# ribal-aladeeb/reinforcement-learning-2048

Measured on AMD Instinct MI355X. Metric: 2048 env steps/sec + DQN updates/sec at 64k parallel boards, 1→8 MI355X, higher is better.
Workload: dtype u8

## Files before the change

reinforcement-learning-2048_amd/csrc/g2048_learn64.hip:

```cpp
#include <hip/hip_runtime.h>
#include <math.h>
#include <stdint.h>
#include <stdlib.h>

#include "../../include/g2048.h"
#include "g2048_board.hpp"
#include "g2048_common.hpp"

namespace {

constexpr int NT = 256;
constexpr int S = 64;
constexpr int XS = 17;
constexpr int HS = 65;
constexpr int P_W1 = 0, P_B1 = 1024, P_W2 = 1088, P_B2 = 1344, P_N = 1348;
constexpr int SLAB = P_N + 4;
constexpr int MAX_SLABS = 256;

struct Net64 {
    double *w1, *b1, *w2, *b2;
};

struct alignas(16) Smem {
    double x[S * XS];
    double h[S * HS];
    double w2[2][4 * 64];
    double b1[2][64];
    double b2[2][4];
    double qa[S * 4];
    double qb[S * 4];
    double y[S];
    double dq[S];
    double loss[S];
    int act[S];
};

__device__ __forceinline__ int64_t sample_row(int64_t b, unsigned long long ep,
                                              unsigned long long count, uint32_t lo, uint32_t hi) {
    const uint4 u = g2048::philox10(
        make_uint4((uint32_t)b, (uint32_t)((uint64_t)b >> 32), (uint32_t)ep,
                   (uint32_t)(ep >> 32) | (g2048::DOMAIN_SAMPLE << 30)),
        lo, hi);
    return (int64_t)__umul64hi(((unsigned long long)u.y << 32) | u.x, count);
}

__device__ __forceinline__ void put_row(double* xr, uint4 v) {
    const uint32_t w[4] = {v.x, v.y, v.z, v.w};
#pragma unroll
    for (int k = 0; k < 4; ++k) {
        xr[4 * k + 0] = (double)(w[k] & 0xFFu);
        xr[4 * k + 1] = (double)((w[k] >> 8) & 0xFFu);
        xr[4 * k + 2] = (double)((w[k] >> 16) & 0xFFu);
        xr[4 * k + 3] = (double)(w[k] >> 24);
    }
}

__device__ __forceinline__ void forward(Smem& M, const double (&w1r)[16], int net, double* q) {
    const int t = threadIdx.x, j = t & 63, rq = t >> 6;
    const double bj = M.b1[net][j];
#pragma unroll 4
    for (int rr = 0; rr < 16; ++rr) {
        const int s = rq * 16 + rr;
        const double* xr = M.x + s * XS;
        double acc = 0.0;
#pragma unroll
        for (int k = 0; k < 16; ++k) acc = fma(w1r[k], xr[k], acc);
        const double pre = acc + bj;
        M.h[s * HS + j] = pre > 0.0 ? pre : 0.0;
    }
    __syncthreads();
    const int s = t >> 2, a = t & 3;
    const double* hr = M.h + s * HS;
    const double* w2 = M.w2[net] + a * 64;
    double acc = 0.0;
#pragma unroll 8
    for (int jj = 0; jj < 64; ++jj) acc = fma(w2[jj], hr[jj], acc);
    q[s * 4 + a] = acc + M.b2[net][a];
    __syncthreads();
}

struct UpdArgs64 {
    Net64 on, tg;
    const uint4 *s, *s2;
    const uint8_t *a, *d;
    const int32_t* r;
    const unsigned long long* count;
    const unsigned long long* step;
    const int64_t* idx_in;
    int64_t batch;
    uint32_t seed_lo, seed_hi;
    float gamma;
    int double_dqn;
    int64_t* idx_out;
    double* y_out;
    double* slab;
    unsigned long long* step_next;
};

typedef uint32_t u32x2 __attribute__((ext_vector_type(2)));
constexpr int AUX_SC1 = 16;
__device__ __forceinline__ __amdgpu_buffer_rsrc_t slab_rsrc(const double* base) {
    return __builtin_amdgcn_make_buffer_rsrc(const_cast<double*>(base), 0, 0x7FFFFFFF, 0x00020000);
}
template <bool COH>
__device__ __forceinline__ void slab_put(double* sl, int e, double v) {
    if constexpr (COH)
        __builtin_amdgcn_raw_buffer_store_b64(__builtin_bit_cast(u32x2, v), slab_rsrc(sl),
                                              (uint32_t)e * 8u, 0u, AUX_SC1);
    else
        sl[e] = v;
}

template <bool COH>
__device__ __forceinline__ void update_tiles64(const UpdArgs64& A) {
    __shared__ Smem M;
    const int t = threadIdx.x, j = t & 63, qd = t >> 6;
    const unsigned long long ep = A.idx_in ? 0ull : *A.step;
    const unsigned long long count = A.idx_in ? 0ull : *A.count;
    if (blockIdx.x == 0 && t == 0) *A.step_next = *A.step + 1ull;
    const Net64 nets[2] = {A.tg, A.on};
    double w1t[16], w1o[16];
#pragma unroll
    for (int k = 0; k < 16; ++k) {
        w1t[k] = A.tg.w1[j * 16 + k];
        w1o[k] = A.on.w1[j * 16 + k];
    }
    for (int i = t; i < 2 * 256; i += NT) M.w2[i >> 8][i & 255] = nets[i >> 8].w2[i & 255];
    if (t < 128) M.b1[t >> 6][t & 63] = nets[t >> 6].b1[t & 63];
    if (t < 8) M.b2[t >> 2][t & 3] = nets[t >> 2].b2[t & 3];
    double w2o[4];
#pragma unroll
    for (int a = 0; a < 4; ++a) w2o[a] = A.on.w2[a * 64 + j];
    double g_w1[4] = {0.0, 0.0, 0.0, 0.0}, g_b1 = 0.0, g_w2 = 0.0, g_b2 = 0.0, g_loss = 0.0;
    const int64_t ntiles = (A.batch + S - 1) / S;
    for (int64_t tile = blockIdx.x; tile < ntiles; tile += gridDim.x) {
        const int64_t b = tile * S + t;
        uint4 sv = make_uint4(0u, 0u, 0u, 0u);
        double rj = 0.0;
        float disc = 0.f;
        bool ok = false;
        __syncthreads();
        if (t < S) {
            uint4 s2v = make_uint4(0u, 0u, 0u, 0u);
            int aj = 0;
            ok = b < A.batch;
            if (ok) {
                const int64_t row =
                    A.idx_in ? A.idx_in[b] : sample_row(b, ep, count, A.seed_lo, A.seed_hi);
                A.idx_out[b] = row;
                s2v = A.s2[row];
                sv = A.s[row];
                aj = A.a[row];
                rj = (double)A.r[row];
                disc = (float)(1 - (int)A.d[row]) * A.gamma;
            }
            put_row(M.x + t * XS, s2v);
            M.act[t] = aj;
        }
        __syncthreads();
        forward(M, w1t, 0, M.qa);
        forward(M, w1o, 1, M.qb);
        if (t < S) {
            const double* qo = M.qb + t * 4;
            const double* qt = M.qa + t * 4;
            double next;
            if (A.double_dqn) {
                const uint32_t as = g2048::argmax4_torch(qo[0], qo[1], qo[2], qo[3]);
                next = qt[as];
            } else {
                next = g2048::qmax4_torch(qt[0], qt[1], qt[2], qt[3]);
            }
            double y;
            {
#pragma clang fp contract(off)
                y = rj + (double)disc * next;
            }
            M.y[t] = y;
            if (ok) A.y_out[b] = y;
            put_row(M.x + t * XS, sv);
        }
        __syncthreads();
        forward(M, w1o, 1, M.qb);
        if (t < S) {
            double dq = 0.0, l = 0.0;
            if (ok) {
#pragma clang fp contract(off)
                const double e = M.qb[t * 4 + M.act[t]] - M.y[t];
                dq = 2.0 * e;
                l = e * e;
            }
            M.dq[t] = dq;
            M.loss[t] = l;
        }
        __syncthreads();
        {
            double acc = 0.0, accb = 0.0;
            for (int s = 0; s < S; ++s) {
                if (M.act[s] == qd) {
                    acc = fma(M.dq[s], M.h[s * HS + j], acc);
                    accb += M.dq[s];
                }
            }
            g_w2 += acc;
            if (j == 0) g_b2 += accb;
        }
        if (t == 0) {
            double l = 0.0;
            for (int s = 0; s < S; ++s) l += M.loss[s];
            g_loss += l;
        }
        __syncthreads();
#pragma unroll 4
        for (int rr = 0; rr < 16; ++rr) {
            const int s = qd * 16 + rr;
            double& hv = M.h[s * HS + j];
            const double w = M.act[s] == 0 ? w2o[0] : M.act[s] == 1 ? w2o[1]
                           : M.act[s] == 2 ? w2o[2] : w2o[3];
            hv = hv > 0.0 ? M.dq[s] * w : 0.0;
        }
        __syncthreads();
        {
            double acc[4] = {0.0, 0.0, 0.0, 0.0}, accb = 0.0;
            for (int s = 0; s < S; ++s) {
                const double dh = M.h[s * HS + j];
                const double* xr = M.x + s * XS + 4 * qd;
#pragma unroll
                for (int i = 0; i < 4; ++i) acc[i] = fma(dh, xr[i], acc[i]);
                accb += dh;
            }
#pragma unroll
            for (int i = 0; i < 4; ++i) g_w1[i] += acc[i];
            if (qd == 0) g_b1 += accb;
        }
    }
    double* sl = A.slab + (int64_t)blockIdx.x * SLAB;
#pragma unroll
    for (int i = 0; i < 4; ++i) slab_put<COH>(sl, P_W1 + j * 16 + 4 * qd + i, g_w1[i]);
    if (qd == 0) slab_put<COH>(sl, P_B1 + j, g_b1);
    slab_put<COH>(sl, P_W2 + qd * 64 + j, g_w2);
    if (j == 0) slab_put<COH>(sl, P_B2 + qd, g_b2);
    if (t == 0) slab_put<COH>(sl, P_N, g_loss);
}

__global__ __launch_bounds__(NT) void k_dense64_update_f64(UpdArgs64 A) { update_tiles64<false>(A); }

constexpr int RW = 16;
static_assert(MAX_SLABS <= RW * 16, "reduction covers at most RW*16 slabs");

struct RedArgs64 {
    const double* slab;
    int nslab;
    double* grad;
    double* loss;
    const unsigned long long* step_next;
    unsigned long long* step;
    double* p[4];
    double* tp[4];
    unsigned long long sync_every;
    double* m;
    double* v;
    double lr, b1, b2, eps;
    int adam;
};

template <int NW, bool COH>
__device__ __forceinline__ void reduce_positions64(const RedArgs64& A, int chunk,
                                                   unsigned long long t, double (*part)[64]) {
    const int lane = threadIdx.x & 63, wave = threadIdx.x >> 6;
    const int pos = chunk * 64 + lane;
    const int k = pos < P_B1 ? 0 : pos < P_W2 ? 1 : pos < P_B2 ? 2 : 3;
    const int base[4] = {P_W1, P_B1, P_W2, P_B2};
    const bool adam = A.adam && wave == 0 && pos < P_N;
    double am = 0.0, av = 0.0, ap = 0.0;
    if (adam) {
        am = A.m[pos];
        av = A.v[pos];
        ap = A.p[k][pos - base[k]];
    }
    constexpr int PW = RW / NW;
    const bool okp = pos <= P_N;
    const int pc = okp ? pos : P_N;
    double v[PW][16];
#pragma unroll
    for (int i = 0; i < PW; ++i)
#pragma unroll
        for (int u = 0; u < 16; ++u) {
            const int g = wave + NW * i + RW * u;
            const bool ok = okp && g < A.nslab;
            const int64_t e = (int64_t)(g < A.nslab ? g : 0) * SLAB + pc;
            double x;
            if constexpr (COH)
                x = __builtin_bit_cast(double, __builtin_amdgcn_raw_buffer_load_b64(
                                                   slab_rsrc(A.slab), (uint32_t)(e * 8), 0u, AUX_SC1));
            else
                x = A.slab[e];
            v[i][u] = ok ? x : 0.0;
        }
#pragma unroll
    for (int i = 0; i < PW; ++i) {
        double r = 0.0;
#pragma unroll
        for (int u = 0; u < 16; ++u) r += v[i][u];
        part[wave + NW * i][lane] = r;
    }
    __syncthreads();
    if (wave == 0 && pos <= P_N) {
        double sum = part[0][lane];
        for (int j = 1; j < RW; ++j) sum += part[j][lane];
        if (pos == P_N) {
            if (A.loss) *A.loss = sum;
        } else {
            if (A.grad) A.grad[pos] = sum;
            if (adam) {
                const double np = g2048::adam64((double)t, A.lr, A.b1, A.b2, A.eps, sum, am, av, ap);
                A.m[pos] = am;
                A.v[pos] = av;
                A.p[k][pos - base[k]] = np;
                if (A.sync_every && t % A.sync_every == 0ull) A.tp[k][pos - base[k]] = np;
            }
        }
    }
}

constexpr int RCHUNKS = (P_N + 1 + 63) / 64;

__global__ __launch_bounds__(64 * RW) void k_dense64_reduce_f64(RedArgs64 A) {
    __shared__ double part[RW][64];
    reduce_positions64<RW, false>(A, blockIdx.x, A.adam ? *A.step_next : 0ull, part);
    if (A.step && blockIdx.x == 0 && threadIdx.x == 0) *A.step = *A.step_next;
}

struct Upd1Args64 {
    UpdArgs64 U;
    RedArgs64 R;
    unsigned int* arrive;
};

__global__ __launch_bounds__(NT) void k_dense64_update1_f64(Upd1Args64 A) {
    const unsigned long long t_next = *A.U.step + 1ull;
    update_tiles64<true>(A.U);
    __shared__ unsigned int s_arrival;
    __shared__ double part[RW][64];
    const unsigned grid = gridDim.x;
    __builtin_amdgcn_s_waitcnt(0);
    __syncthreads();
    if (threadIdx.x == 0)
        s_arrival = __hip_atomic_fetch_add(&A.arrive[0], 1u, __ATOMIC_RELAXED,
                                           __HIP_MEMORY_SCOPE_AGENT);
    __syncthreads();
    const unsigned a = s_arrival;
    const unsigned nred = grid < (unsigned)RCHUNKS ? grid : (unsigned)RCHUNKS;
    if (a >= grid) {
        if (threadIdx.x == 0) atomicAdd(&A.arrive[2], 1u);
        return;
    }
    if (a < grid - nred) return;
    const unsigned me = a - (grid - nred);
    if (threadIdx.x == 0) {
        unsigned it = 0;
        while (__hip_atomic_load(&A.arrive[0], __ATOMIC_RELAXED, __HIP_MEMORY_SCOPE_AGENT) < grid) {
            __builtin_amdgcn_s_sleep(1);
            if (++it == (1u << 24)) {
                atomicAdd(&A.arrive[2], 1u);
                break;
            }
        }
    }
    __syncthreads();
    for (unsigned c = me; c < (unsigned)RCHUNKS; c += nred) {
        reduce_positions64<NT / 64, true>(A.R, (int)c, t_next, part);
        __syncthreads();
    }
    if (threadIdx.x == 0) {
        if (me == 0 && A.R.step) *A.R.step = t_next;
        if (__hip_atomic_fetch_add(&A.arrive[1], 1u, __ATOMIC_RELAXED, __HIP_MEMORY_SCOPE_AGENT) ==
            nred - 1) {
            __hip_atomic_store(&A.arrive[0], 0u, __ATOMIC_RELAXED, __HIP_MEMORY_SCOPE_AGENT);
            __hip_atomic_store(&A.arrive[1], 0u, __ATOMIC_RELAXED, __HIP_MEMORY_SCOPE_AGENT);
        }
    }
}

}

extern "C" G2048_API int64_t g2048_dense64_update_f64_workspace(int64_t batch) {
    const int64_t tiles = (batch + S - 1) / S;
    const int64_t grid = tiles < MAX_SLABS ? tiles : MAX_SLABS;
    return grid * SLAB + 1 + 2;
}

extern "C" G2048_API int g2048_dense64_update_f64(
    const g2048_dense64_params_f64* online, const g2048_dense64_params_f64* target,
    g2048_replay* rb, const int64_t* idx_in, int64_t batch, uint64_t seed, uint64_t* step_dev,
    float gamma, int double_dqn, int64_t* idx_out, double* y_out, double* workspace,
    double* grad_out, double* loss_out, double* exp_avg, double* exp_avg_sq, double lr,
    double beta1, double beta2, double eps, uint64_t sync_every, void* stream) {
    if (!online || !target || !rb || batch <= 0 || !step_dev || !idx_out || !y_out || !workspace)
        return g2048_fail(G2048_EINVAL, "dense64_update_f64: NULL argument or batch <= 0");
    if (!online->w1 || !online->b1 || !online->w2 || !online->b2 || !target->w1 || !target->b1 ||
        !target->w2 || !target->b2)
        return g2048_fail(G2048_EINVAL, "dense64_update_f64: NULL parameter pointer");
    const bool adam = exp_avg && exp_avg_sq;
    if (!adam && !grad_out)
        return g2048_fail(G2048_EINVAL,
                          "dense64_update_f64: need exp_avg and exp_avg_sq (Adam) or grad_out");
    uint8_t *s = nullptr, *s2 = nullptr, *a = nullptr, *d = nullptr;
    int32_t* r = nullptr;
    uint64_t* count = nullptr;
    if (g2048_replay_views(rb, &s, &s2, &a, &r, &d, &count) != G2048_OK) return G2048_EINVAL;
    const int64_t tiles = (batch + S - 1) / S;
    const int grid = (int)(tiles < MAX_SLABS ? tiles : MAX_SLABS);
    UpdArgs64 U;
    U.on = Net64{online->w1, online->b1, online->w2, online->b2};
    U.tg = Net64{target->w1, target->b1, target->w2, target->b2};
    U.s = reinterpret_cast<const uint4*>(s);
    U.s2 = reinterpret_cast<const uint4*>(s2);
    U.a = a;
    U.d = d;
    U.r = r;
    U.count = reinterpret_cast<const unsigned long long*>(count);
    U.step = reinterpret_cast<const unsigned long long*>(step_dev);
    U.idx_in = idx_in;
    U.batch = batch;
    U.seed_lo = (uint32_t)seed;
    U.seed_hi = (uint32_t)(seed >> 32);
    U.gamma = gamma;
    U.double_dqn = double_dqn;
    U.idx_out = idx_out;
    U.y_out = y_out;
    U.slab = workspace;
    U.step_next = reinterpret_cast<unsigned long long*>(workspace + (int64_t)grid * SLAB);
    hipStream_t st = reinterpret_cast<hipStream_t>(stream);
    RedArgs64 R;
    R.slab = workspace;
    R.nslab = grid;
    R.grad = grad_out;
    R.loss = loss_out;
    R.step_next = U.step_next;
    R.step = reinterpret_cast<unsigned long long*>(step_dev);
    double* ps[4] = {online->w1, online->b1, online->w2, online->b2};
    double* ts[4] = {target->w1, target->b1, target->w2, target->b2};
    for (int k = 0; k < 4; ++k) {
        R.p[k] = ps[k];
        R.tp[k] = ts[k];
    }
    R.sync_every = adam ? sync_every : 0ull;
    R.m = exp_avg;
    R.v = exp_avg_sq;
    R.lr = lr;
    R.b1 = beta1;
    R.b2 = beta2;
    R.eps = eps;
    R.adam = adam ? 1 : 0;
    const char* one = getenv("G2048_DENSE64_ONE_LAUNCH");
    if (one && one[0] == '1') {
        Upd1Args64 A1;
        A1.U = U;
        A1.R = R;
        A1.arrive = reinterpret_cast<unsigned int*>(U.step_next + 1);
        hipLaunchKernelGGL(k_dense64_update1_f64, dim3(grid), dim3(NT), 0, st, A1);
    } else {
        hipLaunchKernelGGL(k_dense64_update_f64, dim3(grid), dim3(NT), 0, st, U);
        hipLaunchKernelGGL(k_dense64_reduce_f64, dim3(RCHUNKS), dim3(64 * RW), 0, st, R);
    }
    const hipError_t e = hipGetLastError();
    return e == hipSuccess ? G2048_OK
                           : g2048_fail(G2048_EHIP, "dense64_update_f64: %s", hipGetErrorString(e));
// ... 2 lines not shown
```

reinforcement-learning-2048_amd/csrc/g2048_mlp.hip:

```cpp
#include <hip/hip_runtime.h>
#include <stdint.h>
#include <stdlib.h>

#include "../../include/g2048.h"
#include "g2048_board.hpp"
#include "g2048_common.hpp"

namespace {

constexpr int NT = 256, H = 64;
constexpr int XS = 20, W1S = 17, HS = 68, W2S = 68;
constexpr int S_FWD = 64;
constexpr int S_UPD = 32;
constexpr int P_W1 = 0, P_B1 = 1024, P_W2 = 1088, P_B2 = 1344, P_N = 1348;
constexpr int SLAB = 1352;
constexpr int MAX_SLABS = 256;

struct MlpW {
    const float *w1, *b1, *w2, *b2;
};

struct alignas(16) LW {
    float w1[H * W1S];
    float b1[H];
// ... 342 lines not shown
}

struct UpdateArgs {
    MlpW on, tg;
    const uint8_t *s, *a, *s2, *d;
    const int32_t* r;
    const unsigned long long* count;
    const unsigned long long* step;
    const int64_t* idx_in;
    int64_t batch;
    uint32_t seed_lo, seed_hi;
    float gamma;
    int double_dqn;
    int64_t* idx_out;
    float* y_out;
    float* slab;
    unsigned long long* step_next;
#ifdef G2048_MLP_PHASE
    long long* phase;
#endif
};

#ifdef G2048_MLP_PHASE
#define MPHASE(k) \
    if (threadIdx.x == 0) A.phase[blockIdx.x * 8 + (k)] = __builtin_amdgcn_s_memtime()
#else
#define MPHASE(k)
#endif

template <bool COH>
__device__ __forceinline__ void update_tiles(const UpdateArgs& A) {
    constexpr int S = S_UPD;
    MPHASE(0);
    __shared__ LW Won, Wtg;
    __shared__ Tile<S> T;
    __shared__ float qtg[S * 4];
    const int t = threadIdx.x;
    const unsigned long long ep = A.idx_in ? 0ull : *A.step;
    const unsigned long long count = A.idx_in ? 0ull : *A.count;
    if (blockIdx.x == 0 && t == 0) *A.step_next = *A.step + 1ull;
    stage_weights(A.on, Won);
    stage_weights(A.tg, Wtg);
    const float4 w1on = w1_lane(A.on), w1tg = w1_lane(A.tg);
    GradAcc G;
    const int64_t ntiles = (A.batch + S - 1) / S;
    const int sl = t >> 2, w = t & 3;
    for (int64_t tile = blockIdx.x; tile < ntiles; tile += gridDim.x) {
        const int64_t b0 = tile * S;
        const int64_t b = b0 + sl;
        const bool ok = t < 4 * S && b < A.batch;
        uint32_t s2w = 0, sw = 0;
        int32_t rj = 0;
        uint8_t dj = 0, aj = 0;
        if (ok) {
            const int64_t j =
                A.idx_in ? A.idx_in[b] : sample_row(b, ep, count, A.seed_lo, A.seed_hi);
            s2w = reinterpret_cast<const uint32_t*>(A.s2)[j * 4 + w];
            sw = reinterpret_cast<const uint32_t*>(A.s)[j * 4 + w];
            if (w == 0) {
                A.idx_out[b] = j;
                rj = A.r[j];
                dj = A.d[j];
                aj = A.a[j];
            }
        }
        __syncthreads();
        MPHASE(1);
        if (t < 4 * S) {
            put_word(T.x + sl * XS + w * 4, s2w);
            if (w == 0) {
                T.a[sl] = (float)aj;
                T.g[sl] = ok ? 1.f : 0.f;
            }
        }
        __syncthreads();
        MPHASE(2);
        forward_tile_mfma<S>(T, Wtg, w1tg);
        if (t < 4 * S) qtg[t] = T.q[t];
        forward_tile_mfma<S>(T, Won, w1on);
        if (t < 4 * S && w == 0) {
            const float y = bellman(T.q + sl * 4, qtg + sl * 4, rj, dj, A.gamma, A.double_dqn);
            T.y[sl] = y;
            if (ok) A.y_out[b] = y;
        }
        __syncthreads();
        MPHASE(3);
        if (t < 4 * S) put_word(T.x + sl * XS + w * 4, sw);
        __syncthreads();
        MPHASE(4);
        grad_tile<S>(T, Won, w1on, G);
#ifdef G2048_MLP_PHASE
        __syncthreads();
#endif
        MPHASE(5);
    }
    write_slab<S, COH>(G, T, A.slab + (int64_t)blockIdx.x * SLAB);
    MPHASE(6);
}

__global__ __launch_bounds__(NT) void k_mlp_update(UpdateArgs A) { update_tiles<false>(A); }

constexpr int RW = 16;
static_assert(MAX_SLABS <= RW * 16, "reduction covers at most RW*16 slabs");

struct ReduceArgs {
    const float* slab;
    int nslab;
    float* grad;
    float* loss;
    const unsigned long long* step_next;
    unsigned long long* step;
    float* p[4];
    float* tp[4];
    unsigned long long sync_every;
    float* m;
    float* v;
    double lr, b1, b2, eps;
    int adam;
};

template <int NW, bool COH>
__device__ __forceinline__ void reduce_positions(const ReduceArgs& A, int chunk,
                                                 unsigned long long t, float (*part)[64]) {
    const int lane = threadIdx.x & 63, wave = threadIdx.x >> 6;
    const int pos = chunk * 64 + lane;
    const bool adam = A.adam && wave == 0 && pos < P_N;
    const int k = pos < P_B1 ? 0 : pos < P_W2 ? 1 : pos < P_B2 ? 2 : 3;
    const int base[4] = {P_W1, P_B1, P_W2, P_B2};
    float am = 0.f, av = 0.f, ap = 0.f;
    if (adam) {
        am = A.m[pos];
        av = A.v[pos];
        ap = A.p[k][pos - base[k]];
    }
    constexpr int PW = RW / NW;
    const bool okp = pos <= P_N;
    const int pc = okp ? pos : P_N;
    float r[PW][16];
#pragma unroll
    for (int i = 0; i < PW; ++i)
#pragma unroll
        for (int u = 0; u < 16; ++u) {
            const int g = wave + NW * i + RW * u;
            const bool ok = okp && g < A.nslab;
            const int64_t e = (int64_t)(g < A.nslab ? g : 0) * SLAB + pc;
            float x;
            if constexpr (COH)
                x = __builtin_bit_cast(float, __builtin_amdgcn_raw_buffer_load_b32(
                                                  slab_rsrc(A.slab), (uint32_t)(e * 4), 0u, AUX_SC1));
            else
                x = A.slab[e];
            r[i][u] = ok ? x : 0.f;
        }
#pragma unroll
    for (int i = 0; i < PW; ++i) {
        float v = r[i][0];
#pragma unroll
        for (int u = 1; u < 16; ++u) v += r[i][u];
        part[wave + NW * i][lane] = v;
    }
    __syncthreads();
    if (wave == 0 && pos <= P_N) {
        float sum = part[0][lane];
#pragma unroll
        for (int k2 = 1; k2 < RW; ++k2) sum += part[k2][lane];
        if (pos == P_N) {
            if (A.loss) *A.loss = sum;
        } else {
            if (A.grad) A.grad[pos] = sum;
            if (adam) {
                const g2048::AdamCoef c = g2048::adam_coef((double)t, A.lr, A.b1, A.b2, A.eps);
                const float np = g2048::adam_update(c, sum, am, av, ap);
                A.m[pos] = am;
                A.v[pos] = av;
                A.p[k][pos - base[k]] = np;
                if (A.sync_every && t % A.sync_every == 0ull) A.tp[k][pos - base[k]] = np;
            }
        }
    }
}

constexpr int RCHUNKS = (P_N + 64) / 64;

__global__ __launch_bounds__(64 * RW) void k_mlp_reduce(ReduceArgs A) {
    __shared__ float part[RW][64];
    reduce_positions<RW, false>(A, blockIdx.x, A.adam ? *A.step_next : 0ull, part);
    if (A.step && blockIdx.x == 0 && threadIdx.x == 0) *A.step = *A.step_next;
}

struct Update1Args {
    UpdateArgs U;
    ReduceArgs R;
    unsigned int* arrive;
};

__global__ __launch_bounds__(NT) void k_mlp_update1(Update1Args A) {
    const unsigned long long t_next = *A.U.step + 1ull;
    update_tiles<true>(A.U);
    __shared__ unsigned int s_arrival;
    __shared__ float part[RW][64];
    const unsigned grid = gridDim.x;
    __builtin_amdgcn_s_waitcnt(0);
    __syncthreads();
    if (threadIdx.x == 0)
        s_arrival = __hip_atomic_fetch_add(&A.arrive[0], 1u, __ATOMIC_RELAXED,
                                           __HIP_MEMORY_SCOPE_AGENT);
    __syncthreads();
    const unsigned a = s_arrival;
    const unsigned nred = grid < (unsigned)RCHUNKS ? grid : (unsigned)RCHUNKS;
    if (a >= grid) {
        if (threadIdx.x == 0) atomicAdd(&A.arrive[2], 1u);
        return;
    }
    if (a < grid - nred) return;
    const unsigned me = a - (grid - nred);
    if (threadIdx.x == 0) {
        unsigned it = 0;
        while (__hip_atomic_load(&A.arrive[0], __ATOMIC_RELAXED, __HIP_MEMORY_SCOPE_AGENT) < grid) {
            __builtin_amdgcn_s_sleep(1);
            if (++it == (1u << 24)) {
                atomicAdd(&A.arrive[2], 1u);
                break;
            }
        }
    }
    __syncthreads();
    for (unsigned c = me; c < (unsigned)RCHUNKS; c += nred) {
        reduce_positions<NT / 64, true>(A.R, (int)c, t_next, part);
        __syncthreads();
    }
    if (threadIdx.x == 0) {
        if (me == 0 && A.R.step) *A.R.step = t_next;
        if (__hip_atomic_fetch_add(&A.arrive[1], 1u, __ATOMIC_RELAXED, __HIP_MEMORY_SCOPE_AGENT) ==
            nred - 1) {
            __hip_atomic_store(&A.arrive[0], 0u, __ATOMIC_RELAXED, __HIP_MEMORY_SCOPE_AGENT);
            __hip_atomic_store(&A.arrive[1], 0u, __ATOMIC_RELAXED, __HIP_MEMORY_SCOPE_AGENT);
        }
    }
}

}

namespace {
inline MlpW mlp_w(const g2048_dense64_params* p) { return MlpW{p->w1, p->b1, p->w2, p->b2}; }
inline bool ok_params(const g2048_dense64_params* p) {
    return p && p->w1 && p->b1 && p->w2 && p->b2;
}

}

extern "C" G2048_API int g2048_dense64_forward(const g2048_dense64_params* p, const uint8_t* rows,
                                               const int64_t* idx, int64_t n, float* q_out,
                                               void* stream) {
    if (!ok_params(p) || !rows || !q_out || n <= 0)
        return g2048_fail(G2048_EINVAL, "dense64_forward: NULL argument or n <= 0");
    FwdArgs A{mlp_w(p), rows, idx, n, q_out};
    hipLaunchKernelGGL(k_mlp_forward, dim3((unsigned)((n + S_FWD - 1) / S_FWD)), dim3(NT), 0,
                       reinterpret_cast<hipStream_t>(stream), A);
    const hipError_t e = hipGetLastError();
    return e == hipSuccess ? G2048_OK : g2048_fail(G2048_EHIP, "dense64_forward: %s", hipGetErrorString(e));
}

extern "C" G2048_API int g2048_dense64_targets(const g2048_dense64_params* online,
                                               const g2048_dense64_params* target,
                                               g2048_replay* rb, const int64_t* idx_in,
                                               int64_t batch, uint64_t seed,
                                               const uint64_t* epoch_dev, float gamma,
                                               int double_dqn, int64_t* idx_out, float* y_out,
                                               void* stream) {
    if (!ok_params(online) || !ok_params(target) || !rb || batch <= 0 || !idx_out || !y_out ||
        (!idx_in && !epoch_dev))
        return g2048_fail(G2048_EINVAL, "dense64_targets: NULL argument or batch <= 0");
    uint8_t *s2 = nullptr, *d = nullptr;
    int32_t* r = nullptr;
    uint64_t* count = nullptr;
    if (g2048_replay_views(rb, nullptr, &s2, nullptr, &r, &d, &count) != G2048_OK)
        return G2048_EINVAL;
    TargetArgs A;
    A.on = mlp_w(online);
    A.tg = mlp_w(target);
    A.s2 = s2;
    A.r = r;
    A.d = d;
    A.count = reinterpret_cast<const unsigned long long*>(count);
    A.epoch = reinterpret_cast<const unsigned long long*>(epoch_dev);
    A.idx_in = idx_in;
    A.batch = batch;
    A.seed_lo = (uint32_t)seed;
    A.seed_hi = (uint32_t)(seed >> 32);
    A.gamma = gamma;
    A.double_dqn = double_dqn;
    A.idx_out = idx_out;
    A.y = y_out;
    hipLaunchKernelGGL(k_mlp_targets, dim3((unsigned)((batch + S_FWD - 1) / S_FWD)), dim3(NT), 0,
                       reinterpret_cast<hipStream_t>(stream), A);
    const hipError_t e = hipGetLastError();
    return e == hipSuccess ? G2048_OK : g2048_fail(G2048_EHIP, "dense64_targets: %s", hipGetErrorString(e));
}

extern "C" G2048_API int64_t g2048_dense64_train_workspace(int64_t batch) {
    const int64_t ntiles = (batch + S_FWD - 1) / S_FWD;
    return (ntiles < MAX_SLABS ? ntiles : MAX_SLABS) * SLAB;
}

extern "C" G2048_API int g2048_dense64_train_grad(const g2048_dense64_params* p,
                                                  const uint8_t* rows, const uint8_t* actions,
                                                  const int64_t* idx, const float* y, int64_t batch,
                                                  float* workspace, float* grad_out,
                                                  float* loss_out, uint64_t* step_dev,
                                                  void* stream) {
    if (!ok_params(p) || !rows || !actions || !idx || !y || !workspace || !grad_out || batch <= 0)
        return g2048_fail(G2048_EINVAL, "dense64_train_grad: NULL argument or batch <= 0");
    const int64_t ntiles = (batch + S_FWD - 1) / S_FWD;
    const int grid = (int)(ntiles < MAX_SLABS ? ntiles : MAX_SLABS);
    TrainArgs A{mlp_w(p), rows, actions, idx, y, batch, workspace,
                reinterpret_cast<unsigned long long*>(step_dev)};
    hipStream_t st = reinterpret_cast<hipStream_t>(stream);
    hipLaunchKernelGGL(k_mlp_train, dim3(grid), dim3(NT), 0, st, A);
    hipError_t e = hipGetLastError();
    if (e != hipSuccess) return g2048_fail(G2048_EHIP, "k_mlp_train: %s", hipGetErrorString(e));
    ReduceArgs R{};
    R.slab = workspace;
    R.nslab = grid;
    R.grad = grad_out;
// ... 109 lines not shown
```

reinforcement-learning-2048_amd/g2048/qnet.py:

```python
from __future__ import annotations

import ctypes as C

import torch
from torch import nn

from . import _native as N
from .nets import Conv2048

_CONV_ORDER = ("0.weight", "0.bias", "2.weight", "2.bias", "5.weight", "5.bias", "7.weight",
               "7.bias")
_DENSE_ORDER = ("0.weight", "0.bias", "2.weight", "2.bias")


_DENSE_REF_ORDER = ("0.weight", "0.bias", "2.weight", "2.bias", "4.weight", "4.bias", "6.weight",
                    "6.bias")


def is_dense_ref(model) -> bool:
    dims = [(16, 512), (512, 512), (512, 256), (256, 4)]
    return (isinstance(model, nn.Sequential) and len(model) == 7
            and all(isinstance(model[2 * i], nn.Linear)
                    and (model[2 * i].in_features, model[2 * i].out_features) == d
                    for i, d in enumerate(dims))
# ... 163 lines not shown
        if out is None:
            out = torch.empty((n, 4), dtype=torch.float64, device=rows.device)
        N.check(N.load().g2048_convnet_forward_f64(C.byref(self.p), N.ptr(rows), N.ptr(idx), n,
                                                   N.ptr(out), N.ptr(self.ws),
                                                   N.stream_of(rows.device)),
                "g2048_convnet_forward_f64")
        return out

    def greedy(self, env, epsilon=0.0, eps_schedule=None, out: torch.Tensor | None = None):
        if out is None:
            out = torch.empty((env.n, 4), dtype=torch.float64, device=env.device)
        if out.shape != (env.n, 4) or out.dtype != torch.float64 or not out.is_contiguous():
            raise ValueError(f"out must be a contiguous float64 [{env.n}, 4] tensor")
        eps_ptr, eps_val, dec, mn = env.eps_args(epsilon, eps_schedule)
        N.check(N.load().g2048_convnet_forward_greedy_f64(
            C.byref(self.p), env.handle, eps_ptr, eps_val, dec, mn, N.ptr(out), N.ptr(self.ws),
            N.stream_of(env.device)), "g2048_convnet_forward_greedy_f64")
        return out


class TrainGrad:

    def __init__(self, model, batch: int, adam=None):
        self.kind = kind_of(model)
        self.params = net_params(model)
        self.batch = int(batch)
        self.n_params = sum(p.numel() for p in model.parameters())
        if adam is not None and self.kind != "conv":
            raise TypeError("the Adam-folded reduction exists for the conv net only")
        self.adam = adam
        self._tparams = None
        if adam is not None and adam.sync_every:
            tps = list(adam._target)
            if len(tps) != 8:
                raise ValueError("the attached target must be the conv net's 8 tensors")
            self._tparams = N.ConvNetParams(*[t.data_ptr() for t in tps])
        dev = next(model.parameters()).device
        n = _sym(self.kind, "train_workspace")(self.batch)
        self.workspace = torch.empty(n, dtype=torch.float32, device=dev)

    def __call__(self, rows: torch.Tensor, actions: torch.Tensor, idx: torch.Tensor,
                 y: torch.Tensor, grad_out: torch.Tensor | None, loss_out: torch.Tensor | None = None,
                 step: torch.Tensor | None = None):
        if idx.numel() != self.batch or y.numel() != self.batch:
            raise ValueError("idx / y must have `batch` elements")
        if y.dtype != torch.float32 or (grad_out is not None and (
                grad_out.dtype != torch.float32 or grad_out.numel() != self.n_params)):
            raise ValueError(f"y and grad_out must be float32; grad_out has {self.n_params} elements")
        a = self.adam
        if a is None:
            if grad_out is None:
                raise ValueError("without Adam state the gradient needs a grad_out buffer")
            N.check(_sym(self.kind, "train_grad")(
                C.byref(self.params), N.ptr(rows), N.ptr(actions), N.ptr(idx), N.ptr(y), self.batch,
                N.ptr(self.workspace), N.ptr(grad_out), N.ptr(loss_out), N.ptr(step),
                N.stream_of(rows.device)), "fused train_grad")
            return
        if step is None:
            raise ValueError("the Adam-folded update needs the device step counter")
        tp = C.byref(self._tparams) if self._tparams is not None else None
        N.check(N.load().g2048_convnet_train_adam(
            C.byref(self.params), N.ptr(rows), N.ptr(actions), N.ptr(idx), N.ptr(y), self.batch,
            N.ptr(self.workspace), N.ptr(grad_out), N.ptr(loss_out), N.ptr(step),
            N.ptr(a.exp_avg), N.ptr(a.exp_avg_sq), a.lr, a.betas[0], a.betas[1], a.eps, tp,
            int(a.sync_every) if self._tparams is not None else 0, N.stream_of(rows.device)),
            "g2048_convnet_train_adam")


ConvTrainGrad = TrainGrad


class ConvUpdate:

    def __init__(self, model, target, batch: int, adam=None):
        if kind_of(model) != "conv" or kind_of(target) != "conv":
            raise TypeError("ConvUpdate needs the conv net for online and target")
        self.on, self.tg = net_params(model), net_params(target)
        self.batch = int(batch)
        self.adam = adam
        dev = next(model.parameters()).device
        n = N.load().g2048_convnet_train_workspace(self.batch)
        self.workspace = torch.empty(n, dtype=torch.float32, device=dev)

    def __call__(self, replay, idx_out, y_out, step_dev, gamma=0.8, double_dqn=True, seed=0,
                 idx_in=None, grad_out=None, loss_out=None):
        if idx_out.numel() != self.batch or y_out.numel() != self.batch:
            raise ValueError("idx_out / y_out must have `batch` elements")
        if self.adam is None and grad_out is None:
            raise ValueError("without Adam state the gradient needs a grad_out buffer")
        a = self.adam
        m, v = (a.exp_avg, a.exp_avg_sq) if a is not None else (None, None)
        lr, b1, b2, eps = (a.lr, a.betas[0], a.betas[1], a.eps) if a is not None else (0, 0, 0, 0)
        N.check(N.load().g2048_convnet_update(
            C.byref(self.on), C.byref(self.tg), replay.handle, N.ptr(idx_in), self.batch,
            int(seed), N.ptr(step_dev), float(gamma), int(bool(double_dqn)), N.ptr(idx_out),
            N.ptr(y_out), N.ptr(self.workspace), N.ptr(grad_out), N.ptr(loss_out), N.ptr(m),
            N.ptr(v), float(lr), float(b1), float(b2), float(eps),
            int(a.sync_every) if a is not None else 0, N.stream_of(y_out.device)),
            "g2048_convnet_update")


class Adam64:

    def __init__(self, params, lr: float = 1e-2, betas=(0.9, 0.999), eps: float = 1e-8):
        self.params = list(params)
        self.lr, self.betas, self.eps = float(lr), (float(betas[0]), float(betas[1])), float(eps)
        n = sum(p.numel() for p in self.params)
        dev = self.params[0].device
        self.exp_avg = torch.zeros(n, dtype=torch.float64, device=dev)
        self.exp_avg_sq = torch.zeros(n, dtype=torch.float64, device=dev)
        self.sync_every = 0

        self._ptrs = (C.c_void_p * len(self.params))(*[p.data_ptr() for p in self.params])
        self._numel = (C.c_int64 * len(self.params))(*[p.numel() for p in self.params])
        self._tptrs = None

    def attach_target(self, target_params, sync_every: int) -> None:
        self._target = list(target_params)
        self._tptrs = (C.c_void_p * len(self._target))(*[t.data_ptr() for t in self._target])
        self.sync_every = int(sync_every)

    def reset_state(self):
        self.exp_avg.zero_()
        self.exp_avg_sq.zero_()

    def step(self, grad_flat: torch.Tensor, step_counter: torch.Tensor, grad_scale: float = 1.0):
        lib = N.load()
        args = (self._ptrs, self._numel, len(self.params), N.ptr(grad_flat), N.ptr(self.exp_avg),
                N.ptr(self.exp_avg_sq), N.ptr(step_counter), self.lr, self.betas[0], self.betas[1],
                self.eps, self._tptrs, self.sync_every if self._tptrs is not None else 0)
        if grad_scale == 1.0:
            N.check(lib.g2048_adam_step_sync_f64(*args, N.stream_of(grad_flat.device)),
                    "g2048_adam_step_sync_f64")
        else:
            N.check(lib.g2048_adam_step_scaled_f64(*args, float(grad_scale),
                                                   N.stream_of(grad_flat.device)),
                    "g2048_adam_step_scaled_f64")


class Dense64Update64:

    def __init__(self, model, target, batch: int, adam: Adam64 | None = None):
        if kind64_of(model) != "dense64" or kind64_of(target) != "dense64":
            raise TypeError("Dense64Update64 needs fp64 dense 16-64-4 online and target nets")
        self.on = N.Dense64Params(*[t.data_ptr() for t in
                                    _tensors(model, _DENSE_ORDER, torch.float64)])
        self.tg = N.Dense64Params(*[t.data_ptr() for t in
                                    _tensors(target, _DENSE_ORDER, torch.float64)])
        self.batch = int(batch)
        self.adam = adam
        dev = next(model.parameters()).device
        n = N.load().g2048_dense64_update_f64_workspace(self.batch)
        self.workspace = torch.zeros(n, dtype=torch.float64, device=dev)
        self._grid = min((self.batch + 63) // 64, 256)

    def sync_errors(self) -> int:
        return int(self.workspace[self._grid * 1352 + 1:].view(torch.int32)[2])

    def __call__(self, replay, idx_out, y_out, step_dev, gamma=0.8, double_dqn=True, seed=0,
                 idx_in=None, grad_out=None, loss_out=None):
        if idx_out.numel() != self.batch or y_out.numel() != self.batch:
            raise ValueError("idx_out / y_out must have `batch` elements")
        if y_out.dtype != torch.float64:
            raise TypeError("y_out must be float64")
        if self.adam is None and grad_out is None:
            raise ValueError("without Adam state the gradient needs a grad_out buffer")
        a = self.adam
        m, v = (a.exp_avg, a.exp_avg_sq) if a is not None else (None, None)
        lr, b1, b2, eps = (a.lr, a.betas[0], a.betas[1], a.eps) if a is not None else (0, 0, 0, 0)
        N.check(N.load().g2048_dense64_update_f64(
            C.byref(self.on), C.byref(self.tg), replay.handle, N.ptr(idx_in), self.batch,
            int(seed), N.ptr(step_dev), float(gamma), int(bool(double_dqn)), N.ptr(idx_out),
            N.ptr(y_out), N.ptr(self.workspace), N.ptr(grad_out), N.ptr(loss_out), N.ptr(m),
            N.ptr(v), float(lr), float(b1), float(b2), float(eps),
            int(a.sync_every) if a is not None else 0, N.stream_of(y_out.device)),
            "g2048_dense64_update_f64")


class ConvUpdate64:

    def __init__(self, model, target, batch: int, adam: Adam64 | None = None):
        if kind64_of(model) != "conv" or kind64_of(target) != "conv":
            raise TypeError("ConvUpdate64 needs fp64 Conv2048 online and target nets")
        self._params = (_tensors(model, _CONV_ORDER, torch.float64)
                        + _tensors(target, _CONV_ORDER, torch.float64))
        self.on = N.ConvNetParams(*[t.data_ptr() for t in self._params[:8]])
        self.tg = N.ConvNetParams(*[t.data_ptr() for t in self._params[8:]])
        self.batch = int(batch)
        self.adam = adam
        dev = next(model.parameters()).device
        n = N.load().g2048_convnet_update_f64_workspace(self.batch)
        self.workspace = torch.empty(n, dtype=torch.float64, device=dev)
        self._packed_at = None
        self.ensure_packed()

    def _versions(self):
        return tuple(t._version for t in self._params)

    def ensure_packed(self, force: bool = False) -> bool:
        v = self._versions()
        if not force and v == self._packed_at:
            return False
        N.check(N.load().g2048_convnet_pack_f64(C.byref(self.on), C.byref(self.tg),
                                                N.ptr(self.workspace),
                                                N.stream_of(self.workspace.device)),
                "g2048_convnet_pack_f64")
        self._packed_at = v
        return True

    def __call__(self, replay, idx_out, y_out, step_dev, gamma=0.8, double_dqn=True, seed=0,
                 idx_in=None, grad_out=None, loss_out=None):
        if idx_out.numel() != self.batch or y_out.numel() != self.batch:
            raise ValueError("idx_out / y_out must have `batch` elements")
        if y_out.dtype != torch.float64:
            raise TypeError("y_out must be float64")
        if self.adam is None and grad_out is None:
            raise ValueError("without Adam state the gradient needs a grad_out buffer")
        if not torch.cuda.is_current_stream_capturing():
            self.ensure_packed()
        a = self.adam
        m, v = (a.exp_avg, a.exp_avg_sq) if a is not None else (None, None)
        lr, b1, b2, eps = (a.lr, a.betas[0], a.betas[1], a.eps) if a is not None else (0, 0, 0, 0)
        N.check(N.load().g2048_convnet_update_f64(
            C.byref(self.on), C.byref(self.tg), replay.handle, N.ptr(idx_in), self.batch,
            int(seed), N.ptr(step_dev), float(gamma), int(bool(double_dqn)), N.ptr(idx_out),
            N.ptr(y_out), N.ptr(self.workspace), N.ptr(grad_out), N.ptr(loss_out), N.ptr(m),
            N.ptr(v), float(lr), float(b1), float(b2), float(eps),
            int(a.sync_every) if a is not None else 0, N.stream_of(y_out.device)),
            "g2048_convnet_update_f64")


class DenseRefUpdate:

    def __init__(self, model, target, batch: int, adam=None):
        if not (is_dense_ref(model) and is_dense_ref(target)):
            raise TypeError("DenseRefUpdate needs the reference dense net for online and target")
        dt = next(model.parameters()).dtype
        if dt not in (torch.float32, torch.float64):
            raise TypeError("DenseRefUpdate runs float32 or float64 nets")
        self.dtype = dt
        self.code = N.F32 if dt == torch.float32 else N.F64
        self._params = (_tensors(model, _DENSE_REF_ORDER, dt)
                        + _tensors(target, _DENSE_REF_ORDER, dt))
        self.on = N.DenseNetParams(*[t.data_ptr() for t in self._params[:8]])
        self.tg = N.DenseNetParams(*[t.data_ptr() for t in self._params[8:]])
        self.batch = int(batch)
        self.adam = adam
        dev = next(model.parameters()).device
        n = N.load().g2048_densenet_update_workspace(self.batch, self.code)
        self.workspace = torch.empty(n, dtype=dt, device=dev)

    def __call__(self, replay, idx_out, y_out, step_dev, gamma=0.8, double_dqn=True, seed=0,
                 idx_in=None, grad_out=None, loss_out=None):
        if idx_out.numel() != self.batch or y_out.numel() != self.batch:
            raise ValueError("idx_out / y_out must have `batch` elements")
        if y_out.dtype != self.dtype:
            raise TypeError(f"y_out must be {self.dtype}")
        if self.adam is None and grad_out is None:
            raise ValueError("without Adam state the gradient needs a grad_out buffer")
        a = self.adam
        m, v = (a.exp_avg, a.exp_avg_sq) if a is not None else (None, None)
        lr, b1, b2, eps = (a.lr, a.betas[0], a.betas[1], a.eps) if a is not None else (0, 0, 0, 0)
        N.check(N.load().g2048_densenet_update(
            C.byref(self.on), C.byref(self.tg), self.code, replay.handle, N.ptr(idx_in),
            self.batch, int(seed), N.ptr(step_dev), float(gamma), int(bool(double_dqn)),
            N.ptr(idx_out), N.ptr(y_out), N.ptr(self.workspace), N.ptr(grad_out),
            N.ptr(loss_out), N.ptr(m), N.ptr(v), float(lr), float(b1), float(b2), float(eps),
            int(a.sync_every) if a is not None else 0, N.stream_of(y_out.device)),
            "g2048_densenet_update")


class Dense64Update:

    def __init__(self, model, target, batch: int, adam=None):
        if kind_of(model) != "dense64" or kind_of(target) != "dense64":
            raise TypeError("Dense64Update needs fp32 dense 16-64-4 online and target nets")
        self.on, self.tg = net_params(model), net_params(target)
        self.batch = int(batch)
        self.adam = adam
        dev = next(model.parameters()).device
        n = N.load().g2048_dense64_update_workspace(self.batch)
        self.workspace = torch.zeros(n, dtype=torch.float32, device=dev)
        self._grid = min((self.batch + 31) // 32, 256)

    def sync_errors(self) -> int:
        tail = self.workspace[self._grid * 1352 + 2:].view(torch.int32)
        return int(tail[2])

    def __call__(self, replay, idx_out, y_out, step_dev, gamma=0.8, double_dqn=True, seed=0,
                 idx_in=None, grad_out=None, loss_out=None):
        if idx_out.numel() != self.batch or y_out.numel() != self.batch:
            raise ValueError("idx_out / y_out must have `batch` elements")
        if self.adam is None and grad_out is None:
            raise ValueError("without Adam state the gradient needs a grad_out buffer")
        a = self.adam
        m, v = (a.exp_avg, a.exp_avg_sq) if a is not None else (None, None)
        lr, b1, b2, eps = (a.lr, a.betas[0], a.betas[1], a.eps) if a is not None else (0, 0, 0, 0)
        N.check(N.load().g2048_dense64_update(
            C.byref(self.on), C.byref(self.tg), replay.handle, N.ptr(idx_in), self.batch,
            int(seed), N.ptr(step_dev), float(gamma), int(bool(double_dqn)), N.ptr(idx_out),
            N.ptr(y_out), N.ptr(self.workspace), N.ptr(grad_out), N.ptr(loss_out), N.ptr(m),
            N.ptr(v), float(lr), float(b1), float(b2), float(eps),
            int(a.sync_every) if a is not None else 0, N.stream_of(y_out.device)),
            "g2048_dense64_update")


def targets(kind: str, online, target, replay, batch: int, idx_out: torch.Tensor,
# ... 16 lines not shown
```

Measured before the change: 170.4 billion.

## Fuse the three dense64 forward passes into one tile pass with halved tile size

```diff
diff --git a/reinforcement-learning-2048_amd/csrc/g2048_learn64.hip b/reinforcement-learning-2048_amd/csrc/g2048_learn64.hip
--- a/reinforcement-learning-2048_amd/csrc/g2048_learn64.hip
+++ b/reinforcement-learning-2048_amd/csrc/g2048_learn64.hip
@@ -10,29 +10,34 @@
 namespace {
 
 constexpr int NT = 256;
-constexpr int S = 64;
-constexpr int XS = 17;
-constexpr int HS = 65;
+constexpr int S = 32;
+constexpr int RPW = S / 4;
+constexpr int XS = 16;
+constexpr int HS = 66;
+constexpr int HB = S * HS + 16;
 constexpr int P_W1 = 0, P_B1 = 1024, P_W2 = 1088, P_B2 = 1344, P_N = 1348;
 constexpr int SLAB = P_N + 4;
 constexpr int MAX_SLABS = 256;
+static_assert(NT == 4 * 64 && RPW == 8 && HS % 2 == 0 && HB % 2 == 0, "tile / thread maps");
 
 struct Net64 {
     double *w1, *b1, *w2, *b2;
 };
 
 struct alignas(16) Smem {
-    double x[S * XS];
-    double h[S * HS];
-    double w2[2][4 * 64];
+    double x2[S * XS];
+    double xs[S * XS];
+    double h[3][HB];
+    double w2[2][4 * HS];
     double b1[2][64];
     double b2[2][4];
-    double qa[S * 4];
-    double qb[S * 4];
-    double y[S];
+    double g[4][S];
     double dq[S];
     double loss[S];
+    double r[S];
+    float disc[S];
     int act[S];
+    int ok[S];
 };
 
 __device__ __forceinline__ int64_t sample_row(int64_t b, unsigned long long ep,
@@ -44,39 +49,21 @@
     return (int64_t)__umul64hi(((unsigned long long)u.y << 32) | u.x, count);
 }
 
-__device__ __forceinline__ void put_row(double* xr, uint4 v) {
-    const uint32_t w[4] = {v.x, v.y, v.z, v.w};
-#pragma unroll
-    for (int k = 0; k < 4; ++k) {
-        xr[4 * k + 0] = (double)(w[k] & 0xFFu);
-        xr[4 * k + 1] = (double)((w[k] >> 8) & 0xFFu);
-        xr[4 * k + 2] = (double)((w[k] >> 16) & 0xFFu);
-        xr[4 * k + 3] = (double)(w[k] >> 24);
-    }
-}
-
-__device__ __forceinline__ void forward(Smem& M, const double (&w1r)[16], int net, double* q) {
-    const int t = threadIdx.x, j = t & 63, rq = t >> 6;
-    const double bj = M.b1[net][j];
-#pragma unroll 4
-    for (int rr = 0; rr < 16; ++rr) {
-        const int s = rq * 16 + rr;
-        const double* xr = M.x + s * XS;
-        double acc = 0.0;
-#pragma unroll
-        for (int k = 0; k < 16; ++k) acc = fma(w1r[k], xr[k], acc);
-        const double pre = acc + bj;
-        M.h[s * HS + j] = pre > 0.0 ? pre : 0.0;
-    }
-    __syncthreads();
-    const int s = t >> 2, a = t & 3;
-    const double* hr = M.h + s * HS;
-    const double* w2 = M.w2[net] + a * 64;
-    double acc = 0.0;
-#pragma unroll 8
-    for (int jj = 0; jj < 64; ++jj) acc = fma(w2[jj], hr[jj], acc);
-    q[s * 4 + a] = acc + M.b2[net][a];
-    __syncthreads();
+__device__ __forceinline__ void put_word(double* x, uint32_t w) {
+    double2* x2 = reinterpret_cast<double2*>(x);
+    x2[0] = make_double2((double)(w & 0xFFu), (double)((w >> 8) & 0xFFu));
+    x2[1] = make_double2((double)((w >> 16) & 0xFFu), (double)(w >> 24));
+}
+
+template <int N_>
+__device__ __forceinline__ void lds_read(double (&out)[N_], const double* p) {
+    const double2* p2 = reinterpret_cast<const double2*>(p);
+#pragma unroll
+    for (int i = 0; i < N_ / 2; ++i) {
+        const double2 v = p2[i];
+        out[2 * i] = v.x;
+        out[2 * i + 1] = v.y;
+    }
 }
 
 struct UpdArgs64 {
@@ -118,128 +105,207 @@
     const unsigned long long ep = A.idx_in ? 0ull : *A.step;
     const unsigned long long count = A.idx_in ? 0ull : *A.count;
     if (blockIdx.x == 0 && t == 0) *A.step_next = *A.step + 1ull;
-    const Net64 nets[2] = {A.tg, A.on};
     double w1t[16], w1o[16];
 #pragma unroll
     for (int k = 0; k < 16; ++k) {
         w1t[k] = A.tg.w1[j * 16 + k];
         w1o[k] = A.on.w1[j * 16 + k];
     }
-    for (int i = t; i < 2 * 256; i += NT) M.w2[i >> 8][i & 255] = nets[i >> 8].w2[i & 255];
-    if (t < 128) M.b1[t >> 6][t & 63] = nets[t >> 6].b1[t & 63];
-    if (t < 8) M.b2[t >> 2][t & 3] = nets[t >> 2].b2[t & 3];
+    M.w2[0][qd * HS + j] = A.tg.w2[t];
+    M.w2[1][qd * HS + j] = A.on.w2[t];
+    if (t < 128) M.b1[qd][j] = (qd ? A.on.b1 : A.tg.b1)[j];
+    if (t < 8) M.b2[t >> 2][t & 3] = (t >> 2 ? A.on.b2 : A.tg.b2)[t & 3];
     double w2o[4];
 #pragma unroll
     for (int a = 0; a < 4; ++a) w2o[a] = A.on.w2[a * 64 + j];
     double g_w1[4] = {0.0, 0.0, 0.0, 0.0}, g_b1 = 0.0, g_w2 = 0.0, g_b2 = 0.0, g_loss = 0.0;
     const int64_t ntiles = (A.batch + S - 1) / S;
+    const int sl = t >> 2, w = t & 3;
     for (int64_t tile = blockIdx.x; tile < ntiles; tile += gridDim.x) {
-        const int64_t b = tile * S + t;
-        uint4 sv = make_uint4(0u, 0u, 0u, 0u);
-        double rj = 0.0;
-        float disc = 0.f;
-        bool ok = false;
+        const int64_t b0 = tile * S;
+        const bool ok = t < 4 * S && b0 + sl < A.batch;
+        uint32_t s2w = 0u, sw = 0u;
+        int32_t rj = 0;
+        uint8_t dj = 1, aj = 0;
+        if (ok) {
+            const int64_t b = b0 + sl;
+            const int64_t row =
+                A.idx_in ? A.idx_in[b] : sample_row(b, ep, count, A.seed_lo, A.seed_hi);
+            s2w = reinterpret_cast<const uint32_t*>(A.s2)[row * 4 + w];
+            sw = reinterpret_cast<const uint32_t*>(A.s)[row * 4 + w];
+            if (w == 0) {
+                A.idx_out[b] = row;
+                rj = A.r[row];
+                dj = A.d[row];
+                aj = A.a[row];
+            }
+        }
         __syncthreads();
-        if (t < S) {
-            uint4 s2v = make_uint4(0u, 0u, 0u, 0u);
-            int aj = 0;
-            ok = b < A.batch;
-            if (ok) {
-                const int64_t row =
-                    A.idx_in ? A.idx_in[b] : sample_row(b, ep, count, A.seed_lo, A.seed_hi);
-                A.idx_out[b] = row;
-                s2v = A.s2[row];
-                sv = A.s[row];
-                aj = A.a[row];
-                rj = (double)A.r[row];
-                disc = (float)(1 - (int)A.d[row]) * A.gamma;
-            }
-            put_row(M.x + t * XS, s2v);
-            M.act[t] = aj;
+        if (t < 4 * S) {
+            put_word(M.x2 + sl * XS + 4 * w, s2w);
+            put_word(M.xs + sl * XS + 4 * w, sw);
+            if (w == 0) {
+                M.act[sl] = aj & 3;
+                M.ok[sl] = ok ? 1 : 0;
+                M.r[sl] = (double)rj;
+                M.disc[sl] = (float)(1 - (int)dj) * A.gamma;
+            }
         }
         __syncthreads();
-        forward(M, w1t, 0, M.qa);
-        forward(M, w1o, 1, M.qb);
-        if (t < S) {
-            const double* qo = M.qb + t * 4;
-            const double* qt = M.qa + t * 4;
+        {
+            const double bt = M.b1[0][j], bo = M.b1[1][j];
+#pragma unroll 4
+            for (int rr = 0; rr < RPW; ++rr) {
+                const int s = qd * RPW + rr;
+                double x2[16], xs[16];
+                lds_read(x2, M.x2 + s * XS);
+                lds_read(xs, M.xs + s * XS);
+                double at = 0.0, ao = 0.0, as = 0.0;
+#pragma unroll
+                for (int k = 0; k < 16; ++k) {
+                    at = fma(w1t[k], x2[k], at);
+                    ao = fma(w1o[k], x2[k], ao);
+                    as = fma(w1o[k], xs[k], as);
+                }
+                const double pt = at + bt, po = ao + bo, ps = as + bo;
+                M.h[0][s * HS + j] = pt > 0.0 ? pt : 0.0;
+                M.h[1][s * HS + j] = po > 0.0 ? po : 0.0;
+                M.h[2][s * HS + j] = ps > 0.0 ? ps : 0.0;
+            }
+        }
+        __syncthreads();
+        {
+            const int net = j >> 5, r = (j >> 2) & 7, a = j & 3;
+            const int s = qd * RPW + r;
+            const double* h1 = M.h[net] + s * HS;
+            const double* h2 = M.h[2] + s * HS;
+            const double* wa = M.w2[net] + a * HS;
+            const double* wb = M.w2[1] + a * HS;
+            double q1 = 0.0, q2 = 0.0;
+#pragma unroll 2
+            for (int j0 = 0; j0 < 64; j0 += 8) {
+                double hv1[8], hv2[8], wv1[8], wv2[8];
+                lds_read(hv1, h1 + j0);
+                lds_read(wv1, wa + j0);
+                lds_read(hv2, h2 + j0);
+                lds_read(wv2, wb + j0);
+#pragma unroll
+                for (int i = 0; i < 8; ++i) {
+                    q1 = fma(wv1[i], hv1[i], q1);
+                    q2 = fma(wv2[i], hv2[i], q2);
+                }
+            }
+            q1 += M.b2[net][a];
+            q2 += M.b2[1][a];
+            double qt[4], qo[4];
+#pragma unroll
+            for (int i = 0; i < 4; ++i) {
+                qt[i] = __shfl(q1, 4 * r + i);
+                qo[i] = __shfl(q1, 32 + 4 * r + i);
+            }
             double next;
             if (A.double_dqn) {
                 const uint32_t as = g2048::argmax4_torch(qo[0], qo[1], qo[2], qo[3]);
-                next = qt[as];
+                const double lo = as & 1u ? qt[1] : qt[0], hi = as & 1u ? qt[3] : qt[2];
+                next = as & 2u ? hi : lo;
             } else {
                 next = g2048::qmax4_torch(qt[0], qt[1], qt[2], qt[3]);
             }
             double y;
             {
 #pragma clang fp contract(off)
-                y = rj + (double)disc * next;
-            }
-            M.y[t] = y;
-            if (ok) A.y_out[b] = y;
-            put_row(M.x + t * XS, sv);
-        }
-        __syncthreads();
-        forward(M, w1o, 1, M.qb);
-        if (t < S) {
-            double dq = 0.0, l = 0.0;
-            if (ok) {
+                y = M.r[s] + (double)M.disc[s] * next;
+            }
+            if (net == 0) {
+                const int act = M.act[s];
+                const bool oks = M.ok[s] != 0;
+                double dq = 0.0, l = 0.0;
+                if (oks) {
 #pragma clang fp contract(off)
-                const double e = M.qb[t * 4 + M.act[t]] - M.y[t];
-                dq = 2.0 * e;
-                l = e * e;
-            }
-            M.dq[t] = dq;
-            M.loss[t] = l;
+                    const double e = q2 - y;
+                    dq = 2.0 * e;
+                    l = e * e;
+                }
+                M.g[a][s] = a == act ? dq : 0.0;
+                if (a == act) {
+                    M.dq[s] = dq;
+                    M.loss[s] = l;
+                    if (oks) A.y_out[b0 + s] = y;
+                }
+            }
         }
         __syncthreads();
         {
             double acc = 0.0, accb = 0.0;
-            for (int s = 0; s < S; ++s) {
-                if (M.act[s] == qd) {
-                    acc = fma(M.dq[s], M.h[s * HS + j], acc);
-                    accb += M.dq[s];
+#pragma unroll
+            for (int s0 = 0; s0 < S; s0 += 16) {
+                double gs[16], hv[16];
+                lds_read(gs, M.g[qd] + s0);
+#pragma unroll
+                for (int i = 0; i < 16; ++i) hv[i] = M.h[2][(s0 + i) * HS + j];
+#pragma unroll
+                for (int i = 0; i < 16; ++i) {
+                    acc = fma(gs[i], hv[i], acc);
+                    accb += gs[i];
                 }
             }
             g_w2 += acc;
             if (j == 0) g_b2 += accb;
         }
-        if (t == 0) {
-            double l = 0.0;
-            for (int s = 0; s < S; ++s) l += M.loss[s];
+        if (qd == 0) {
+            double l = M.loss[j & (S - 1)];
+#pragma unroll
+            for (int off = S / 2; off > 0; off >>= 1) l += __shfl_xor(l, off);
             g_loss += l;
         }
-        __syncthreads();
-#pragma unroll 4
-        for (int rr = 0; rr < 16; ++rr) {
-            const int s = qd * 16 + rr;
-            double& hv = M.h[s * HS + j];
-            const double w = M.act[s] == 0 ? w2o[0] : M.act[s] == 1 ? w2o[1]
-                           : M.act[s] == 2 ? w2o[2] : w2o[3];
-            hv = hv > 0.0 ? M.dq[s] * w : 0.0;
+        {
+            double dq[RPW], hv[RPW];
+            int act[RPW];
+            lds_read(dq, M.dq + qd * RPW);
+#pragma unroll
+            for (int rr = 0; rr < RPW; ++rr) {
+                act[rr] = M.act[qd * RPW + rr];
+                hv[rr] = M.h[2][(qd * RPW + rr) * HS + j];
+            }
+#pragma unroll
+            for (int rr = 0; rr < RPW; ++rr) {
+                const double lo = act[rr] & 1 ? w2o[1] : w2o[0], hi = act[rr] & 1 ? w2o[3] : w2o[2];
+                const double wv = act[rr] & 2 ? hi : lo;
+                const long long keep = hv[rr] > 0.0 ? -1ll : 0ll;
+                M.h[0][(qd * RPW + rr) * HS + j] =
+                    __longlong_as_double(__double_as_longlong(dq[rr] * wv) & keep);
+            }
         }
         __syncthreads();
         {
             double acc[4] = {0.0, 0.0, 0.0, 0.0}, accb = 0.0;
-            for (int s = 0; s < S; ++s) {
-                const double dh = M.h[s * HS + j];
-                const double* xr = M.x + s * XS + 4 * qd;
-#pragma unroll
-                for (int i = 0; i < 4; ++i) acc[i] = fma(dh, xr[i], acc[i]);
-                accb += dh;
+#pragma unroll 2
+            for (int s0 = 0; s0 < S; s0 += 8) {
+                double dh[8], xr[8][4];
+#pragma unroll
+                for (int i = 0; i < 8; ++i) {
+                    dh[i] = M.h[0][(s0 + i) * HS + j];
+                    lds_read(xr[i], M.xs + (s0 + i) * XS + 4 * qd);
+                }
+#pragma unroll
+                for (int i = 0; i < 8; ++i) {
+#pragma unroll
+                    for (int c = 0; c < 4; ++c) acc[c] = fma(dh[i], xr[i][c], acc[c]);
+                    accb += dh[i];
+                }
             }
 #pragma unroll
             for (int i = 0; i < 4; ++i) g_w1[i] += acc[i];
             if (qd == 0) g_b1 += accb;
         }
     }
-    double* sl = A.slab + (int64_t)blockIdx.x * SLAB;
-#pragma unroll
-    for (int i = 0; i < 4; ++i) slab_put<COH>(sl, P_W1 + j * 16 + 4 * qd + i, g_w1[i]);
-    if (qd == 0) slab_put<COH>(sl, P_B1 + j, g_b1);
-    slab_put<COH>(sl, P_W2 + qd * 64 + j, g_w2);
-    if (j == 0) slab_put<COH>(sl, P_B2 + qd, g_b2);
-    if (t == 0) slab_put<COH>(sl, P_N, g_loss);
+    double* slab = A.slab + (int64_t)blockIdx.x * SLAB;
+#pragma unroll
+    for (int i = 0; i < 4; ++i) slab_put<COH>(slab, P_W1 + j * 16 + 4 * qd + i, g_w1[i]);
+    if (qd == 0) slab_put<COH>(slab, P_B1 + j, g_b1);
+    slab_put<COH>(slab, P_W2 + qd * 64 + j, g_w2);
+    if (j == 0) slab_put<COH>(slab, P_B2 + qd, g_b2);
+    if (t == 0) slab_put<COH>(slab, P_N, g_loss);
 }
 
 __global__ __launch_bounds__(NT) void k_dense64_update_f64(UpdArgs64 A) { update_tiles64<false>(A); }
@@ -296,6 +362,8 @@
                 x = A.slab[e];
             v[i][u] = ok ? x : 0.0;
         }
+    g2048::Adam64Coef cf{0.0, 0.0};
+    if (A.adam && wave == 0) cf = g2048::adam64_coef((double)t, A.lr, A.b1, A.b2);
 #pragma unroll
     for (int i = 0; i < PW; ++i) {
         double r = 0.0;
@@ -312,7 +380,7 @@
         } else {
             if (A.grad) A.grad[pos] = sum;
             if (adam) {
-                const double np = g2048::adam64((double)t, A.lr, A.b1, A.b2, A.eps, sum, am, av, ap);
+                const double np = g2048::adam64_apply(cf, A.b1, A.b2, A.eps, sum, am, av, ap);
                 A.m[pos] = am;
                 A.v[pos] = av;
                 A.p[k][pos - base[k]] = np;
diff --git a/reinforcement-learning-2048_amd/csrc/g2048_mlp.hip b/reinforcement-learning-2048_amd/csrc/g2048_mlp.hip
--- a/reinforcement-learning-2048_amd/csrc/g2048_mlp.hip
+++ b/reinforcement-learning-2048_amd/csrc/g2048_mlp.hip
@@ -518,6 +518,8 @@
                 x = A.slab[e];
             r[i][u] = ok ? x : 0.f;
         }
+    g2048::AdamCoef c{};
+    if (A.adam && wave == 0) c = g2048::adam_coef((double)t, A.lr, A.b1, A.b2, A.eps);
 #pragma unroll
     for (int i = 0; i < PW; ++i) {
         float v = r[i][0];
@@ -535,7 +537,6 @@
         } else {
             if (A.grad) A.grad[pos] = sum;
             if (adam) {
-                const g2048::AdamCoef c = g2048::adam_coef((double)t, A.lr, A.b1, A.b2, A.eps);
                 const float np = g2048::adam_update(c, sum, am, av, ap);
                 A.m[pos] = am;
                 A.v[pos] = av;
diff --git a/reinforcement-learning-2048_amd/g2048/qnet.py b/reinforcement-learning-2048_amd/g2048/qnet.py
--- a/reinforcement-learning-2048_amd/g2048/qnet.py
+++ b/reinforcement-learning-2048_amd/g2048/qnet.py
@@ -339,7 +339,7 @@
         dev = next(model.parameters()).device
         n = N.load().g2048_dense64_update_f64_workspace(self.batch)
         self.workspace = torch.zeros(n, dtype=torch.float64, device=dev)
-        self._grid = min((self.batch + 63) // 64, 256)
+        self._grid = min((self.batch + 31) // 32, 256)
 
     def sync_errors(self) -> int:
         return int(self.workspace[self._grid * 1352 + 1:].view(torch.int32)[2])
```

Result: no change. 170.3 billion (-0.1%).
